# gsgen3d/gsgen

Hardware: AMD Instinct MI355X
Metric: fwd+bwd renders/sec (800x800, 100k Gaussians) (higher is better)
Workload: dtype f32

## Files before the change

gsgen_amd/csrc/common.hpp:

```cpp
#pragma once
#include <hip/hip_runtime.h>
#include <stdint.h>

#if defined(__clang__)
#define GS_WAVES_PER_EU(n) __attribute__((amdgpu_waves_per_eu(n)))
#else
#define GS_WAVES_PER_EU(n)
#endif

namespace gs {

constexpr int kTile = 16;
constexpr int kListOverflow = -2;
constexpr float kMinAlpha = 0.00392156862745098f;
constexpr float kAlphaClamp = 0.99f;
constexpr float kLog2e = 1.4426950408889634f;
constexpr float kGuardTol = 2.0e-4f;
constexpr float kInvSc2 = 1.3862943611198906f;

__device__ __forceinline__ int lane_id() { return (int)(threadIdx.x & 63u); }

struct CholRec { float p0, p1, p2; bool ok; };
__device__ __forceinline__ CholRec chol_prep(float c0, float c1, float c2, float c3) {
#pragma clang fp contract(off)
// ... 14 lines not shown
}

typedef float v2f __attribute__((vector_size(8)));

__device__ __forceinline__ float wave_sum(float v) {
#pragma unroll
  for (int m = 32; m >= 1; m >>= 1) v += __shfl_xor(v, m, 64);
  return v;
}

__device__ __forceinline__ bool wave_any(bool pred) {
#if defined(__HIP_DEVICE_COMPILE__)
  return __builtin_amdgcn_ballot_w64(pred) != 0ull;
#else
  return __ballot((int)pred) != 0ull;
#endif
}
__device__ __forceinline__ void wave_mem_fence() {
#if defined(__HIP_DEVICE_COMPILE__)
  __builtin_amdgcn_fence(__ATOMIC_RELEASE, "workgroup");
  __builtin_amdgcn_wave_barrier();
  __builtin_amdgcn_fence(__ATOMIC_ACQUIRE, "workgroup");
#else
  (void)__ballot(1);
#endif
}
__device__ __forceinline__ float wave_uniform(float v) {
  return __int_as_float(__builtin_amdgcn_readfirstlane(__float_as_int(v)));
}

// ... 346 lines not shown
```

gsgen_amd/csrc/composite.hip:

```cpp
#include "composite_common.hpp"
#include <stdio.h>
#include <string.h>
#include <string>
#include <type_traits>
#include <vector>

namespace gs {

template <int MODE, int CB, int KB = kBatch, bool WITH_COL = true>
struct Stage {
  using TR = Traits<MODE, CB>;
  float mx[KB], my[KB], a[KB];
  float c0[KB], c1[KB], c2[KB], c3[KB];
  float p0[KB], p1[KB], p2[KB];
  int id[KB];
  alignas(16) float col[WITH_COL ? KB * TR::NCOLP : 4];
};

template <int MODE, int CB, int NT, int KB = kBatch, bool SCALE = false, bool WITH_COL = true>
__device__ __forceinline__ void stage_batch(Stage<MODE, CB, KB, WITH_COL> &S, const CompParams &p, int list_base,
                                            int nb) {
  using TR = Traits<MODE, CB>;
  const int t = (int)threadIdx.x;
  static_assert(KB <= NT, "one thread per staged record");
// ... 124 lines not shown
  CompParams v[kPackMax];
  __host__ __device__ const CompParams *table() const { return v; }
};
template <> struct ViewPack<false> {
  __host__ __device__ const CompParams *table() const { return nullptr; }
};
__device__ __forceinline__ uint32_t batch_view(const CompParams &p_arg, uint32_t &bid, uint32_t *grid, uint32_t total) {
  const uint32_t B = (uint32_t)p_arg.n_lo, per = total / B;
  const uint32_t view = bid / per;
  bid -= view * per;
  if (grid) *grid = per;
  return view;
}
__device__ __forceinline__ uint32_t batch_view(const CompParams &p_arg, uint32_t &bid, uint32_t *grid = nullptr) {
  return batch_view(p_arg, bid, grid, gridDim.x);
}

template <int MODE, int CB, int PPL, int TS = 16>
__global__ void __launch_bounds__(TS * TS / PPL) k_composite_fwd(CompParams p) {
  const uint32_t bid = blockIdx.x;
  using TR = Traits<MODE, CB>;
  constexpr int NT = TS * TS / PPL;
  constexpr int ROWS = NT / TS;
  static_assert(TS == 8 || TS == 16 || TS == 32, "tile side");
  static_assert(NT >= kBatch && NT % 64 == 0, "a staging round needs one thread per record");
  constexpr int NCH = TR::NCH;
  __shared__ Stage<MODE, CB> S;

  int tx, ty;
  if (!block_tile(p, tx, ty, bid)) return;
// ... 252 lines not shown
    lg[2][j >> 1][j & 1] = l.s2;
  }
}
template <int NP>
__device__ __forceinline__ void poly_rows_at_pixels(const float *cg, v2f pu2, const v2f (&pv2)[NP], v2f (&yv)[3][NP]) {
#pragma unroll
  for (int c = 0; c < 3; ++c) {
    const float *cw = cg + c * kPolyStride;
    const v2f ab = ffma2(pu2, ffma2(pu2, *reinterpret_cast<const v2f *>(cw + 4), *reinterpret_cast<const v2f *>(cw + 2)),
                         *reinterpret_cast<const v2f *>(cw));
    const float Cc = cw[6];
#pragma unroll
    for (int jp = 0; jp < NP; ++jp) yv[c][jp] = ffma2(pv2[jp], ffma2(pv2[jp], splat2(Cc), splat2(ab[1])), splat2(ab[0]));
  }
}
template <int NT>
__device__ __forceinline__ uint32_t exact_tier_mask(const CompParams &p, const int *ids, int nb, int t, uint32_t *slot) {
  bool bad = false;
  if (p.sh_rows != nullptr && t < nb) bad = !poly_row_ok(p.sh_rows[ids[t]], fmaxf(fabsf(p.psx), fabsf(p.psy)));
  const uint32_t m = (uint32_t)__ballot((int)bad);
  if constexpr (NT == 64) {
    (void)slot;
    return m;
  } else {
    if (t == 0) *slot = m;
    return 0u;
  }
}
template <int CB, bool POLY>
struct FwdShVecShared {
  static constexpr int KB = POLY ? 32 : kBatch;
  Stage<MODE_SH, CB, KB, !POLY> S;
  alignas(16) float Vs[POLY ? kPolyNB * 16 : 4];
  alignas(16) float Ws[POLY ? KB * 3 * kPolyStride : 4];
  uint32_t exact_mask;
  float tay_ok[POLY ? KB * 3 : 1];
};
template <int CB, int PPL, int NB, bool PERSIST = false, bool TRACK = true>
__device__ __forceinline__ void composite_fwd_sh_vec_tile(const CompParams &p, uint32_t bid, FwdShVecShared<CB, (NB > 0)> &sm) {
  static_assert(PPL == 4 || PPL == 2, "pixel pairs: 2 or 4 pixels per lane");
  constexpr bool POLY = NB > 0;
  static_assert(!POLY || (NB == kPolyNB && CB == 4), "polynomial basis: SH degree 3");
  constexpr int MODE = MODE_SH;
  using TR = Traits<MODE, CB>;
  constexpr int NT = 256 / PPL, ROWS = NT / 16, NP = PPL / 2;
  constexpr int CCP = POLY ? NB : TR::CCP, NPAIR = CCP / 2;
  constexpr int KB = FwdShVecShared<CB, POLY>::KB;
  auto &S = sm.S;
  float *const Vs = sm.Vs;
  float *const Ws = sm.Ws;
  int tx, ty;
  if (!block_tile(p, tx, ty, bid)) return;
  const int tile = ty * p.ntw + tx;
  const int st = p.start[tile];
  const int n = (st < 0) ? 0 : (p.end[tile] - st);
  const int t = tile_thread_index<PERSIST>();
  const int lx = t & 15, ly0 = t >> 4;
  const int gx = tx * kTile + lx;

  bool valid[PPL];
  int gy[PPL], stop[PPL];
#pragma unroll
  for (int j = 0; j < PPL; ++j) {
    gy[j] = ty * kTile + ly0 + j * ROWS;
    valid[j] = (gx < p.W) && (gy[j] < p.H);
    stop[j] = valid[j] ? n : 0;
  }
// ... 60 lines not shown
#pragma unroll
  for (int jp = 0; jp < NP; ++jp) {
#pragma unroll
    for (int c = 0; c < 3; ++c) acc2[jp][c] = v2f{0.0f, 0.0f};
    Tr2[jp] = v2f{valid[2 * jp] ? 1.0f : -1.0f, valid[2 * jp + 1] ? 1.0f : -1.0f};
  }
  auto alive = [&](int j) { return !(Tr2[j >> 1][j & 1] < p.thresh); };
  const bool seg_out = p.nseg > 1 && p.ckpt != nullptr;
  const bool track_stop = TRACK && p.stop != nullptr;

  uint32_t exact_mask = 0u;
  uint32_t tay_mask = 0u;
  for (int base = 0; base < n; base += KB) {
    const int nb = min(KB, n - base);
    if (base > 0) __syncthreads();
    stage_batch<MODE, CB, NT, KB, true, !POLY>(S, p, st + base, nb);
    if constexpr (POLY) {
      if (p.sh_rows != nullptr) {
        exact_mask = exact_tier_mask<NT>(p, S.id, nb, t, &sm.exact_mask);
        __syncthreads();
        if constexpr (NT != 64) exact_mask = sm.exact_mask;
        exact_mask = (uint32_t)__builtin_amdgcn_readfirstlane((int)exact_mask);
        if (__popcll((unsigned long long)exact_mask) * kExactTierShare > nb) {
          if (t == 0 && p.route_report != nullptr) report_crowded_tile(p.route_report);
          if (!p.no_fallback) {
            if (t == 0 && p.tile_flags != nullptr) p.tile_flags[tile] = 1;
            return;
          }
        }
      } else {
        exact_mask = 0u;
        __syncthreads();
      }
      poly_transform<NT, KB>(p.col, S.id, Vs, Ws, nb, sm.tay_ok);
      __syncthreads();
      tay_mask = (uint32_t)__builtin_amdgcn_readfirstlane((int)(taylor_mask(sm.tay_ok, nb) & ~exact_mask));
      taylor_convert<NT>(Ws, tay_mask, nb);
      __syncthreads();
    } else {
      __syncthreads();
    }

    for (int g = 0; g < nb; ++g) {
      bool any_alive = false;
#pragma unroll
      for (int j = 0; j < PPL; ++j) any_alive |= alive(j);
      if (!wave_any(any_alive)) break;
      const int e_idx = base + g;
      if (seg_out && (e_idx % kSegLen) == 0 && e_idx > 0 && e_idx / kSegLen < p.nseg) {
#pragma unroll
        for (int j = 0; j < PPL; ++j)
          p.ckpt[((size_t)tile * p.nseg + e_idx / kSegLen) * 256 + (ly0 + j * ROWS) * 16 + lx] =
              make_float4(Tr2[j >> 1][j & 1], acc2[j >> 1][0][j & 1], acc2[j >> 1][1][j & 1], acc2[j >> 1][2][j & 1]);
      }
// ... 186 lines not shown
}
template <int CB, int PPL, bool BATCH = false, int NB = 0, bool TRACK = true, bool PSD = false>
__global__ void __launch_bounds__(256 / PPL)
GS_WAVES_PER_EU((NB == kPolyNB && BATCH && PPL == 4 && !TRACK) ? 5 : 1)
k_composite_fwd_sh_vec(CompParams p_arg, ViewPack<BATCH> pack) {
  static_assert(!PSD || (BATCH && NB != kRouted), "pixel sizes from device memory: the batched launches' three shapes");
  const CompParams *plist = pack.table();
  uint32_t bid = blockIdx.x;
  if constexpr (NB == kRouted) {
    static_assert(CB == 4, "routing exists for SH degree 3");
    union Shared {
      FwdShVecShared<4, true> poly;
      FwdShVecShared<4, false> exact;
    };
    __shared__ Shared sm;
    const CompParams *pp = BATCH ? &plist[batch_view(p_arg, bid)] : &p_arg;
    const bool poly = routed_tile_is_polynomial(*pp, bid);
    if (poly) {
      CompParams p = *pp;
      p.sh_rows = nullptr;
      composite_fwd_sh_vec_tile<4, PPL, kPolyNB>(p, bid, sm.poly);
    } else {
      const CompParams p = *pp;
      composite_fwd_sh_vec_tile<4, PPL, 0>(p, bid, sm.exact);
    }
  } else if constexpr (NB == kFallback) {
    static_assert(CB == 4 && BATCH, "the persistent exact fallback of a bounded batch");
    __shared__ FwdShVecShared<4, false> sm;
    const uint32_t B = (uint32_t)p_arg.n_lo, total = p_arg.vgrid;
    const bool per_tile = plist[0].sh_rows != nullptr;
    if (!per_tile) {
// ... 6 lines not shown
    }
    const uint32_t per = total / B;
    uint32_t base = 0;
    uint32_t view = 0;
    for (uint32_t b = blockIdx.x; b < total; b += gridDim.x) {
      while (b >= base + per) { base += per; ++view; }
      const CompParams *pp = &plist[view];
      const PixelSizes<PSD> ps = view_pixel_sizes<PSD>(*pp);
      if (per_tile ? !tile_flagged(*pp, b - base) : poly_route(pp->sh_bound, ps.x(), ps.y())) continue;
      const CompParams p = view_params<PSD>(*pp, ps);
      composite_fwd_sh_vec_tile<4, PPL, 0, true>(p, b - base, sm);
      __syncthreads();
    }
  } else if constexpr (NB == kPolyNB && BATCH) {
    __shared__ FwdShVecShared<4, true> sm;
    const CompParams *pp = &plist[batch_view(p_arg, bid)];
    const PixelSizes<PSD> ps = view_pixel_sizes<PSD>(*pp);
    const bool view_ok = pp->sh_bound != nullptr && poly_route(pp->sh_bound, ps.x(), ps.y());
    if (pp->sh_rows == nullptr && !view_ok) return;
    CompParams p = view_params<PSD>(*pp, ps);
    if (view_ok) p.sh_rows = nullptr;
    composite_fwd_sh_vec_tile<4, PPL, kPolyNB, false, TRACK>(p, bid, sm);
  } else {
    const CompParams *pp = BATCH ? &plist[batch_view(p_arg, bid)] : &p_arg;
    const CompParams p = view_params<PSD>(*pp, view_pixel_sizes<PSD>(*pp));
    __shared__ FwdShVecShared<CB, (NB > 0)> sm;
    composite_fwd_sh_vec_tile<CB, PPL, NB>(p, bid, sm);
  }
}

template <int MODE, int CB, int PPL, int TS>
__global__ void __launch_bounds__(TS * TS / PPL)
k_composite_bwd_pixel(CompParams p) {
  const uint32_t bid = blockIdx.x, grid = gridDim.x;
  using TR = Traits<MODE, CB>;
  constexpr int NT = TS * TS / PPL;
  static_assert(NT >= kBatch && NT % 64 == 0, "a staging round needs one thread per record");
  constexpr int ROWS = NT / TS;
  constexpr int NCH = TR::NCH;
// ... 207 lines not shown
    for (int j = 0; j < PPL; ++j) any_alive |= alive[j];
    if (__syncthreads_or((int)any_alive) == 0) break;
  }
}


template <int CB, int PPL, bool POLY>
struct BwdShVecShared {
  static constexpr int KB = 32;
  static constexpr int NT = 256 / PPL, NP = PPL / 2;
  Stage<MODE_SH, CB, KB, !POLY> S;
  v2f go_s[!POLY ? 3 * NP * NT : 1];
  alignas(16) float Vs[POLY ? kPolyNB * 16 : 4];
  alignas(16) float Ws[POLY ? KB * 3 * kPolyStride : 4];
  float gw_s[POLY ? 3 * 8 : 1];
  float tay_ok[POLY ? KB * 3 : 1];
};
template <int CB, int PPL, int NB, bool PERSIST = false, bool MOM = false>
__device__ __forceinline__ void composite_bwd_sh_vec_tile(const CompParams &p, uint32_t bid, uint32_t grid,
                                                          BwdShVecShared<CB, PPL, (NB > 0)> &sm) {
  static_assert(PPL == 4 || PPL == 2, "pixel pairs: 2 or 4 pixels per lane");
  constexpr bool POLY = NB > 0;
  static_assert(!POLY || (NB == kPolyNB && CB == 4 && PPL == 4), "polynomial basis: SH degree 3, one wavefront per tile");
  constexpr int MODE = MODE_SH;
  using TR = Traits<MODE, CB>;
  constexpr int NT = 256 / PPL, ROWS = NT / 16, NP = PPL / 2;
  constexpr int CCP = POLY ? NB : TR::CCP, NPAIR = CCP / 2, NSH = 3 * CCP;
  static_assert(NSH % 2 == 0, "component layout");
  constexpr int KB = BwdShVecShared<CB, PPL, POLY>::KB;
  auto &S = sm.S;
  v2f *const go_s = sm.go_s;
  float *const Vs = sm.Vs;
  float *const Ws = sm.Ws;
  float *const gw_s = sm.gw_s;
  const int nseg = p.nseg > 1 ? p.nseg : 1;
  const uint32_t tiles_grid = grid / (uint32_t)nseg;
  const int seg = (int)(bid / tiles_grid);
  int tx, ty;
  if (!block_tile(p, tx, ty, bid % tiles_grid)) return;
  const int tile = ty * p.ntw + tx;
  const int st = p.start[tile];
  const int n = (st < 0) ? 0 : (p.end[tile] - st);
  if (n == 0 || n < p.n_lo || n >= p.n_hi) return;
  if constexpr (POLY) {
    if (p.tile_flags != nullptr && p.tile_flags[tile] != 0) return;
  }
  const int e_lo = seg * kSegLen;
  const int e_hi = (seg == nseg - 1) ? n : min(n, e_lo + kSegLen);
  if (e_lo >= n) return;
  const int t = tile_thread_index<PERSIST>();
  const int lane = t & 63;
  const int lx = t & 15, ly0 = t >> 4;
  const int gx = tx * kTile + lx;
  const float px = pixel_coord(p.topleft[0], gx, p.psx);
// ... 81 lines not shown
    R2[jp] = fma2(go2[jp][2], rem2[jp][2], fma2(go2[jp][1], rem2[jp][1], go2[jp][0] * rem2[jp][0]));
    pvsq2[jp] = pv2[jp] * pv2[jp];
  }
  if constexpr (!POLY) {
#pragma unroll
    for (int jp = 0; jp < NP; ++jp)
#pragma unroll
      for (int c = 0; c < 3; ++c) go_s[(c * NP + jp) * NT + t] = go2[jp][c];
  }
  auto alive = [&](int j) { return !(Tr2[j >> 1][j & 1] < p.thresh); };

  uint32_t exact_mask = 0u, tay_mask = 0u;
  for (int base = e_lo; base < e_hi; base += KB) {
    const int nb = min(KB, e_hi - base);
    if (base > e_lo) __syncthreads();
    stage_batch<MODE, CB, NT, KB, true, !POLY>(S, p, st + base, nb);
    __syncthreads();
    if constexpr (POLY) {
      exact_mask = (uint32_t)__builtin_amdgcn_readfirstlane((int)exact_tier_mask<NT>(p, S.id, nb, t, nullptr));
      poly_transform<NT, KB>(p.col, S.id, Vs, Ws, nb, sm.tay_ok);
      __syncthreads();
      tay_mask = (uint32_t)__builtin_amdgcn_readfirstlane((int)(taylor_mask(sm.tay_ok, nb) & ~exact_mask));
      taylor_convert<NT>(Ws, tay_mask, nb);
      __syncthreads();
    }

    for (int g = 0; g < nb; ++g) {
      bool any_alive = false;
#pragma unroll
      for (int j = 0; j < PPL; ++j) any_alive |= alive(j);
      if (!wave_any(any_alive)) break;

      auto uni = [&](float v) { return !POLY ? wave_uniform(v) : v; };
      const float r_mx = uni(S.mx[g]), r_my = uni(S.my[g]), r_a = uni(S.a[g]), r_c0 = uni(S.c0[g]), r_c1 = uni(S.c1[g]),
                  r_c2 = uni(S.c2[g]), r_c3 = uni(S.c3[g]), r_p0 = uni(S.p0[g]), r_p1 = uni(S.p1[g]);
      const float x = px - r_mx;
      v2f y2[NP], G2[NP], ag2[NP], tx2[NP], ty2[NP];
      bool any_con = false;
      float guard_dist = 0.0f;
#pragma unroll
// ... 224 lines not shown
template <int CB, int PPL, bool BATCH = false, int NB = 0, bool MOM = false, bool PSD = false>
__global__ void __launch_bounds__(256 / PPL)
GS_WAVES_PER_EU((NB == kPolyNB && BATCH) ? 4 : 1)
k_composite_bwd_sh_vec(CompParams p_arg, ViewPack<BATCH> pack) {
  static_assert(!MOM || (BATCH && NB != kRouted), "the moment form exists for the batched launches");
  static_assert(!PSD || (BATCH && NB != kRouted), "pixel sizes from device memory: the batched launches' three shapes");
  const CompParams *plist = pack.table();
  uint32_t bid = blockIdx.x, grid = gridDim.x;
  if constexpr (NB == kRouted) {
    static_assert(CB == 4 && PPL == 4, "routing exists for SH degree 3, one wavefront per tile");
    union Shared {
      BwdShVecShared<4, 4, true> poly;
      BwdShVecShared<4, 4, false> exact;
    };
    __shared__ Shared sm;
    const CompParams *pp = BATCH ? &plist[batch_view(p_arg, bid, &grid)] : &p_arg;
    const uint32_t tiles_grid = grid / (uint32_t)(pp->nseg > 1 ? pp->nseg : 1);
    const bool poly = routed_tile_is_polynomial(*pp, bid % tiles_grid);
    if (poly) {
      CompParams p = *pp;
      p.sh_rows = nullptr;
      composite_bwd_sh_vec_tile<4, 4, kPolyNB>(p, bid, grid, sm.poly);
    } else {
      const CompParams p = *pp;
      composite_bwd_sh_vec_tile<4, 4, 0>(p, bid, grid, sm.exact);
    }
  } else if constexpr (NB == kFallback) {
    static_assert(CB == 4 && PPL == 4 && BATCH, "the persistent exact fallback of a bounded batch");
    __shared__ BwdShVecShared<4, 4, false> sm;
    const uint32_t B = (uint32_t)p_arg.n_lo, total = p_arg.vgrid;
    const bool per_tile = plist[0].sh_rows != nullptr;
// ... 8 lines not shown
    const uint32_t per = total / B;
    const uint32_t tiles_grid = per / (uint32_t)(plist[0].nseg > 1 ? plist[0].nseg : 1);
    uint32_t base = 0;
    uint32_t view = 0;
    for (uint32_t b = blockIdx.x; b < total; b += gridDim.x) {
      while (b >= base + per) { base += per; ++view; }
      const CompParams *pp = &plist[view];
      const PixelSizes<PSD> ps = view_pixel_sizes<PSD>(*pp);
      if (per_tile ? !tile_flagged(*pp, (b - base) % tiles_grid) : poly_route(pp->sh_bound, ps.x(), ps.y())) continue;
      const CompParams p = view_params<PSD>(*pp, ps);
      composite_bwd_sh_vec_tile<4, 4, 0, true, MOM>(p, b - base, per, sm);
      __syncthreads();
    }
  } else if constexpr (NB == kPolyNB && BATCH) {
    __shared__ BwdShVecShared<4, 4, true> sm;
    const CompParams *pp = &plist[batch_view(p_arg, bid, &grid)];
    const PixelSizes<PSD> ps = view_pixel_sizes<PSD>(*pp);
    const bool view_ok = pp->sh_bound != nullptr && poly_route(pp->sh_bound, ps.x(), ps.y());
    if (pp->sh_rows == nullptr && !view_ok) return;
    CompParams p = view_params<PSD>(*pp, ps);
    if (view_ok) p.sh_rows = nullptr;
    composite_bwd_sh_vec_tile<4, 4, kPolyNB, false, MOM>(p, bid, grid, sm);
  } else {
    const CompParams *pp = BATCH ? &plist[batch_view(p_arg, bid, &grid)] : &p_arg;
    const CompParams p = view_params<PSD>(*pp, view_pixel_sizes<PSD>(*pp));
    __shared__ BwdShVecShared<CB, PPL, (NB > 0)> sm;
    composite_bwd_sh_vec_tile<CB, PPL, NB, false, MOM>(p, bid, grid, sm);
  }
}

template <int MODE, bool BATCH = false>
__global__ void __launch_bounds__(64) GS_WAVES_PER_EU(6)
k_composite_fwd_chan_vec(CompParams p_arg, ViewPack<BATCH> pack) {
  const CompParams *plist = pack.table();
  static_assert(MODE == MODE_RGB || MODE == MODE_SCALAR || MODE == MODE_RGBD, "post-activation channel modes");
  uint32_t bid = blockIdx.x;
  const CompParams p = BATCH ? view_params(plist[batch_view(p_arg, bid)]) : p_arg;
  using TR = Traits<MODE, 1>;
  constexpr int PPL = 4, NT = 64, ROWS = NT / 16, NP = PPL / 2;
// ... 402 lines not shown
template <int MODE, int CB>
static int launch_fwd(const CompParams &p_, hipStream_t s) {
  CompParams p = p_;
  const uint32_t nblk = comp_grid(p);
  if (p.ntw * p.nth == 0) return 0;
  if (p.tile_side != 16) {
    if constexpr (MODE == MODE_RGBD) return GSGEN_EUNSUPPORTED;
    else {
      if (p.nseg > 1) return GSGEN_EUNSUPPORTED;
      p.sh_bound = p.sh_rows = nullptr;
      if (p.tile_side == 8) hipLaunchKernelGGL((k_composite_fwd<MODE, CB, 1, 8>), dim3(nblk), dim3(64), 0, s, p);
      else hipLaunchKernelGGL((k_composite_fwd<MODE, CB, 4, 32>), dim3(nblk), dim3(256), 0, s, p);
      return (int)hipGetLastError();
    }
  }
  if constexpr (MODE == MODE_SH && CB == 4) {
    if (p.sh_bound != nullptr || p.sh_rows != nullptr) {
      hipLaunchKernelGGL((k_composite_fwd_sh_vec<4, 2, false, kRouted>), dim3(nblk), dim3(128), 0, s, p, ViewPack<false>{});
      return (int)hipGetLastError();
    }
  } else {
    p.sh_bound = p.sh_rows = nullptr;
  }
  hipLaunchKernelGGL((k_composite_fwd<MODE, CB, 1>), dim3(nblk), dim3(256), 0, s, p);
  return (int)hipGetLastError();
}
template <int MODE, int CB>
static int launch_bwd(const CompParams &p_, hipStream_t s) {
  CompParams p = p_;
  if (p.n_hi == 0) p.n_hi = 0x7fffffff;
  const uint32_t nblk = comp_grid(p);
  if (p.ntw * p.nth == 0) return 0;
  if (p.tile_side != 16) {
    if constexpr (MODE == MODE_RGBD) return GSGEN_EUNSUPPORTED;
    else {
      if (p.nseg > 1) return GSGEN_EUNSUPPORTED;
      p.sh_bound = p.sh_rows = nullptr;
      if (p.tile_side == 8) hipLaunchKernelGGL((k_composite_bwd_pixel<MODE, CB, 1, 8>), dim3(nblk), dim3(64), 0, s, p);
      else hipLaunchKernelGGL((k_composite_bwd_pixel<MODE, CB, 4, 32>), dim3(nblk), dim3(256), 0, s, p);
      return (int)hipGetLastError();
    }
  }
  if constexpr (MODE != MODE_SH) {
    p.sh_bound = nullptr;
    hipLaunchKernelGGL((k_composite_bwd_chan_vec<MODE>), dim3(nblk), dim3(64), 0, s, p, ViewPack<false>{});
  } else {
    const uint32_t ng = nblk * (uint32_t)(p.nseg > 1 ? p.nseg : 1);
    if constexpr (CB == 4) {
      if (p.sh_bound != nullptr || p.sh_rows != nullptr) {
        hipLaunchKernelGGL((k_composite_bwd_sh_vec<4, 4, false, kRouted>), dim3(ng), dim3(64), 0, s, p, ViewPack<false>{});
        return (int)hipGetLastError();
      }
    } else {
      p.sh_bound = p.sh_rows = nullptr;
    }
    hipLaunchKernelGGL((k_composite_bwd_sh_vec<CB, 4>), dim3(ng), dim3(64), 0, s, p, ViewPack<false>{});
  }
  return (int)hipGetLastError();
}


static ViewPack<true> make_pack(const CompParams *host, uint32_t n) {
  ViewPack<true> pack{};
  for (uint32_t i = 0; i < n; ++i) pack.v[i] = host[i];
  return pack;
}
template <class F>
static void for_each_chunk(const CompParams *host, uint32_t B, F &&f) {
  for (uint32_t b0 = 0; b0 < B; b0 += (uint32_t)kPackMax) {
    const uint32_t n = (B - b0) < (uint32_t)kPackMax ? (B - b0) : (uint32_t)kPackMax;
    CompParams a = host[b0];
    a.n_lo = (int)n;
    f(a, make_pack(host + b0, n), n);
  }
}
template <int CB, bool PSD>
static void launch_fwd_sh_batch_c(const CompParams &p0, const ViewPack<true> &plist, uint32_t B, uint32_t nblk, hipStream_t s, bool bounded) {
  const dim3 g(nblk * B);
  if constexpr (CB == 4) {
    if (bounded) {
      CompParams pf = p0;
      pf.vgrid = nblk * B;
      const uint32_t gf = pf.vgrid < 2560u ? pf.vgrid : 2560u;
      const auto fallback = [&] { hipLaunchKernelGGL((k_composite_fwd_sh_vec<4, 2, true, kFallback, true, PSD>), dim3(gf), dim3(128), 0, s, pf, plist); };
      const auto polynomial = [&] {
        if (p0.stop == nullptr) hipLaunchKernelGGL((k_composite_fwd_sh_vec<4, 4, true, kPolyNB, false, PSD>), g, dim3(64), 0, s, p0, plist);
        else hipLaunchKernelGGL((k_composite_fwd_sh_vec<4, 4, true, kPolyNB, true, PSD>), g, dim3(64), 0, s, p0, plist);
// ... 3 lines not shown
        if (!p0.no_fallback) fallback();
        return;
      }
      fallback();
      polynomial();
      return;
    }
  }
  hipLaunchKernelGGL((k_composite_fwd_sh_vec<CB, 2, true, 0, true, PSD>), g, dim3(128), 0, s, p0, plist);
}
template <bool PSD>
static int launch_fwd_sh_batch_p(int C, const CompParams *host, uint32_t B, hipStream_t s, bool bounded) {
  if (B == 0 || host[0].ntw * host[0].nth == 0) return 0;
  const uint32_t nblk = comp_grid(host[0]);
  const bool poly = C == 4 && bounded;
  for_each_chunk(host, B, [&](const CompParams &p0, const ViewPack<true> &pack, uint32_t n) {
    switch (C) {
      case 1: launch_fwd_sh_batch_c<1, PSD>(p0, pack, n, nblk, s, false); break;
      case 2: launch_fwd_sh_batch_c<2, PSD>(p0, pack, n, nblk, s, false); break;
      case 3: launch_fwd_sh_batch_c<3, PSD>(p0, pack, n, nblk, s, false); break;
      default: launch_fwd_sh_batch_c<4, PSD>(p0, pack, n, nblk, s, poly); break;
    }
  });
  return (int)hipGetLastError();
}
int launch_fwd_sh_batch(int C, const CompParams *host, uint32_t B, hipStream_t s, bool bounded) {
  return (B != 0 && host[0].ps_dev != nullptr) ? launch_fwd_sh_batch_p<true>(C, host, B, s, bounded)
                                               : launch_fwd_sh_batch_p<false>(C, host, B, s, bounded);
}
template <int CB, bool MOM, bool PSD>
static void launch_bwd_sh_batch_c(const CompParams &p0, const ViewPack<true> &plist, uint32_t B, uint32_t nblk, hipStream_t s, bool bounded) {
// ... 4 lines not shown
      pf.vgrid = nblk * B;
      const uint32_t gf = pf.vgrid < 3072u ? pf.vgrid : 3072u;
      if (!(p0.sh_rows != nullptr && p0.no_fallback))
        hipLaunchKernelGGL((k_composite_bwd_sh_vec<4, 4, true, kFallback, MOM, PSD>), dim3(gf), dim3(64), 0, s, pf, plist);
      hipLaunchKernelGGL((k_composite_bwd_sh_vec<4, 4, true, kPolyNB, MOM, PSD>), g, dim3(64), 0, s, p0, plist);
      return;
    }
  }
  hipLaunchKernelGGL((k_composite_bwd_sh_vec<CB, 4, true, 0, MOM, PSD>), g, dim3(64), 0, s, p0, plist);
}
template <bool MOM, bool PSD>
static int launch_bwd_sh_batch_m(int C, const CompParams *host, uint32_t B, hipStream_t s, bool bounded) {
  if (B == 0 || host[0].ntw * host[0].nth == 0) return 0;
  const uint32_t nblk = comp_grid(host[0]) * (uint32_t)(host[0].nseg > 1 ? host[0].nseg : 1);
  const bool poly = C == 4 && bounded;
  for_each_chunk(host, B, [&](const CompParams &p0, const ViewPack<true> &pack, uint32_t n) {
    switch (C) {
      case 1: launch_bwd_sh_batch_c<1, MOM, PSD>(p0, pack, n, nblk, s, false); break;
      case 2: launch_bwd_sh_batch_c<2, MOM, PSD>(p0, pack, n, nblk, s, false); break;
      case 3: launch_bwd_sh_batch_c<3, MOM, PSD>(p0, pack, n, nblk, s, false); break;
      default: launch_bwd_sh_batch_c<4, MOM, PSD>(p0, pack, n, nblk, s, poly); break;
    }
  });
  return (int)hipGetLastError();
}
int launch_bwd_sh_batch(int C, const CompParams *host, uint32_t B, hipStream_t s, bool bounded, bool moments = false) {
  if (B != 0 && host[0].ps_dev != nullptr)
    return moments ? launch_bwd_sh_batch_m<true, true>(C, host, B, s, bounded) : launch_bwd_sh_batch_m<false, true>(C, host, B, s, bounded);
  return moments ? launch_bwd_sh_batch_m<true, false>(C, host, B, s, bounded) : launch_bwd_sh_batch_m<false, false>(C, host, B, s, bounded);
}

template <int MODE, bool MOM = false>
static int launch_chan_batch(bool backward, const CompParams *host, uint32_t B, hipStream_t s) {
  if (B == 0 || host[0].ntw * host[0].nth == 0) return 0;
  const uint32_t nblk = comp_grid(host[0]);
  for_each_chunk(host, B, [&](const CompParams &p0, const ViewPack<true> &pack, uint32_t n) {
    if (backward) hipLaunchKernelGGL((k_composite_bwd_chan_vec<MODE, true, MOM>), dim3(nblk * n), dim3(64), 0, s, p0, pack);
    else hipLaunchKernelGGL((k_composite_fwd_chan_vec<MODE, true>), dim3(nblk * n), dim3(64), 0, s, p0, pack);
  });
  return (int)hipGetLastError();
}
int launch_fwd_rgbd_batch(const CompParams *host, uint32_t B, hipStream_t s) { return launch_chan_batch<MODE_RGBD>(false, host, B, s); }
int launch_bwd_rgbd_batch(const CompParams *host, uint32_t B, hipStream_t s) { return launch_chan_batch<MODE_RGBD>(true, host, B, s); }
int launch_bwd_rgbd_batch_moments(const CompParams *host, uint32_t B, hipStream_t s) { return launch_chan_batch<MODE_RGBD, true>(true, host, B, s); }
int launch_fwd_rgb_batch(const CompParams *host, uint32_t B, hipStream_t s) { return launch_chan_batch<MODE_RGB>(false, host, B, s); }
int launch_bwd_rgb_batch(const CompParams *host, uint32_t B, hipStream_t s) { return launch_chan_batch<MODE_RGB>(true, host, B, s); }

int launch_bwd_pixel_dispatch(int mode, int C, const CompParams &p, hipStream_t s) {
  if (mode == MODE_RGB) return launch_bwd<MODE_RGB, 1>(p, s);
  if (mode == MODE_SCALAR) return launch_bwd<MODE_SCALAR, 1>(p, s);
  if (mode == MODE_RGBD) return launch_bwd<MODE_RGBD, 1>(p, s);
// ... 643 lines not shown
```

gsgen_amd/csrc/composite_common.hpp:

```cpp
#pragma once
#include "common.hpp"
#include "../../include/gsgen_hip.h"

namespace gs {

enum : int { MODE_RGB = 0, MODE_SCALAR = 1, MODE_SH = 2, MODE_RGBD = 3 };
constexpr int kBatch = 64;

struct CompParams {
  const float *mean, *cov, *col, *alpha;
  const float *depth;
  const int *start, *end, *ids;
  const float *topleft, *rot, *bg;
  float *out, *T;
  const float *final_img, *grad_out;
  float *g_mean, *g_cov, *g_col, *g_alpha;
  int ntw, nth, H, W;
  float psx, psy, thresh;
  const uint32_t *tile_order;
  int n_lo, n_hi;
  float4 *ckpt;
  int *stop;
  int nseg;
  int tile_side;
  const float *go_rgb, *go_d, *go_o, *go_z2;
  const float *sh_bound;
  const float *sh_rows;
  uint8_t *tile_flags;
  uint32_t vgrid;
  int fill_empty;
  float *pl_rgb, *pl_d, *pl_o, *pl_z;
  float *g_bg;
  int zvar;
  const float *chol;
  uint32_t *route_report;
  int no_fallback;
  const float *ps_dev;
};
__device__ __forceinline__ CompParams view_params(const CompParams &src) {
  CompParams p = src;
  if (p.ps_dev != nullptr) {
    p.psx = p.ps_dev[0];
    p.psy = p.ps_dev[1];
  }
  return p;
}
constexpr int kSegLen = 32;

__device__ __forceinline__ bool block_tile(const CompParams &p, int &tx, int &ty, uint32_t bid) {
  if (p.tile_order != nullptr) {
    const uint32_t t = p.tile_order[bid];
    tx = (int)(t % (uint32_t)p.ntw);
    ty = (int)(t / (uint32_t)p.ntw);
    return true;
  }
  return tile_of_block(bid, p.ntw, p.nth, tx, ty);
}
__device__ __forceinline__ bool block_tile(const CompParams &p, int &tx, int &ty) {
  return block_tile(p, tx, ty, blockIdx.x);
}
__host__ __forceinline__ uint32_t comp_grid(const CompParams &p) {
  return p.tile_order != nullptr ? (uint32_t)(p.ntw * p.nth) : tile_map_blocks(p.ntw, p.nth);
}

static __device__ __noinline__ float gauss_ref_f64(float mx, float my, float c0f, float c1f, float c2f,
                                            float c3f, float px, float py) {
  const double c0 = c0f, c1 = c1f, c2 = c2f, c3 = c3f;
  const double det = c0 * c3 - c1 * c2;
  const double x = (double)(px - mx);
  const double y = (double)(py - my);
  const double tx = x * c3 - y * c2;
  const double ty = -x * c1 + y * c0;
  double radial = tx * x + ty * y;
  radial /= det;
// ... 261 lines not shown
  if (t < 16) {
    float y[kPolyNodes];
#pragma unroll
    for (int n = 0; n < kPolyNodes; ++n) y[n] = Yn[n * 16 + t];
#pragma unroll
    for (int r = 0; r < kPolyNB; ++r) {
      float acc = 0.0f;
#pragma unroll
      for (int n = 0; n < kPolyNodes; ++n)
        if (kPolyFit[r][n] != 0.0f) acc = fmaf(kPolyFit[r][n], y[n], acc);
      Vs[r * 16 + t] = acc;
    }
  }
  __syncthreads();
}
template <int NT, int KB>
__device__ __forceinline__ void poly_transform(const float *__restrict__ sh, const int *ids, const float *Vs, float *w, int nb,
                                               float *tay_ok ) {
  static_assert(NT % 2 == 0, "the two halves of a row sit in neighbouring lanes");
#pragma unroll 1
  for (int it0 = 0; it0 < nb * 6; it0 += NT) {
    const int it = it0 + (int)threadIdx.x;
    const bool live = it < nb * 6;
    const int e = live ? (it >> 1) : 0, half = it & 1;
    const int g = e / 3, c = e - 3 * g;
    const float4 *q4 = reinterpret_cast<const float4 *>(sh + (size_t)ids[g] * 48 + c * 16);
    const float4 q0 = q4[0], q1 = q4[1], q2 = q4[2], q3 = q4[3];
    const v2f qa = {q0.x, q0.y}, qb = {q0.z, q0.w}, qc = {q1.x, q1.y}, qd = {q1.z, q1.w}, qe = {q2.x, q2.y}, qf = {q2.z, q2.w},
              qg = {q3.x, q3.y}, qh = {q3.z, q3.w};
    float *row = w + e * kPolyStride;
    const int s0 = half ? 6 : 0, s1 = half ? 3 : 1, s2 = half ? 4 : 2;
#pragma unroll 1
    for (int k = 0; k < 3; ++k) {
      const float4 *v4 = reinterpret_cast<const float4 *>(Vs + (3 * half + k) * 16);
      const float4 a = v4[0], b = v4[1], cc = v4[2], d = v4[3];
      v2f acc = qa * v2f{a.x, a.y};
      acc = ffma2(qb, v2f{a.z, a.w}, acc);
      acc = ffma2(qc, v2f{b.x, b.y}, acc);
      acc = ffma2(qd, v2f{b.z, b.w}, acc);
      acc = ffma2(qe, v2f{cc.x, cc.y}, acc);
      acc = ffma2(qf, v2f{cc.z, cc.w}, acc);
      acc = ffma2(qg, v2f{d.x, d.y}, acc);
      acc = ffma2(qh, v2f{d.z, d.w}, acc);
      if (live) row[k == 0 ? s0 : (k == 1 ? s1 : s2)] = -kLog2e * (acc[0] + acc[1]);
    }
    if (live && !half) row[5] = 0.0f;
    const float mine = live ? fabsf(row[s0]) + fabsf(row[s1]) + fabsf(row[s2]) : 0.0f;
    const float l1 = xor_add<1>(mine);
    if (live && l1 > 40.0f) {
      const float sc = 40.0f / l1;
      row[s0] *= sc; row[s1] *= sc; row[s2] *= sc;
    }
    if (live && !half) {
      const float l = mine - fabsf(row[0]), q = l1 - mine;
      tay_ok[e] = (l1 <= 40.0f && taylor_row_ok(l, q)) ? 1.0f : 0.0f;
    }
  }
}
template <int NT>
__device__ __forceinline__ void taylor_convert(float *w, uint32_t mask, int nb) {
#pragma unroll 1
  for (int e = (int)threadIdx.x; e < nb * 3; e += NT) {
    if (!((mask >> (e / 3)) & 1u)) continue;
    float *row = w + e * kPolyStride;
    const float w1 = row[1], w2 = row[2], w4 = row[3], w5 = row[4], w3 = row[6];
    const float f0 = __builtin_amdgcn_rcpf(1.0f + __builtin_amdgcn_exp2f(row[0]));
    const float ff = f0 * (1.0f - f0);
    const float f1 = -0.6931471805599453f * ff, f2 = 0.2402265069591007f * ff * (1.0f - 2.0f * f0);
    row[0] = f0;
    row[1] = f1 * w1;
    row[2] = f1 * w2;
    row[3] = fmaf(f1, w4, 2.0f * f2 * w1 * w2);
    row[4] = fmaf(f1, w5, f2 * w2 * w2);
    row[6] = fmaf(f1, w3, f2 * w1 * w1);
  }
}
__device__ __forceinline__ uint32_t taylor_mask(const float *tay_ok, int nb) {
  const int l = lane_id();
  const bool ok = l < nb && tay_ok[3 * l] != 0.0f && tay_ok[3 * l + 1] != 0.0f && tay_ok[3 * l + 2] != 0.0f;
  return (uint32_t)__ballot((int)ok);
}

static inline int check_common(uint32_t tile_size, const void *a, const void *b, const void *c) {
  if (tile_size < 1u || tile_size > 32u) return GSGEN_EUNSUPPORTED;
  if (!a || !b || !c) return GSGEN_EINVAL;
  return 0;
}

}
```

Measured before the change: 7515.

## Fuse polynomial staging, SH transform and Taylor conversion into one wave pass

Replaces the separate stage_batch, exact-tier mask, poly_transform and taylor_convert phases with a single poly_stage_batch. In it, one wavefront handles 32 records using a lane pair per record, and the masks come from ballots instead of shared-memory flags. This removes several __syncthreads barriers and shared-memory round trips per batch. Separately, it precomputes reciprocal multipliers on the host so that block-to-tile and batch-view integer divisions become multiply-shift. The cost is that only 64 threads do the staging work in 128-thread blocks, which may serialize work that was spread before.

New measurement: 7574 (median of 6 runs). Within noise of the previous version (+0.8%).

```diff
diff --git a/gsgen_amd/csrc/common.hpp b/gsgen_amd/csrc/common.hpp
--- a/gsgen_amd/csrc/common.hpp
+++ b/gsgen_amd/csrc/common.hpp
@@ -52,6 +52,13 @@
   return __builtin_amdgcn_ballot_w64(pred) != 0ull;
 #else
   return __ballot((int)pred) != 0ull;
+#endif
+}
+__device__ __forceinline__ unsigned long long wave_ballot(bool pred) {
+#if defined(__HIP_DEVICE_COMPILE__)
+  return __builtin_amdgcn_ballot_w64(pred);
+#else
+  return __ballot((int)pred);
 #endif
 }
 __device__ __forceinline__ void wave_mem_fence() {
diff --git a/gsgen_amd/csrc/composite.hip b/gsgen_amd/csrc/composite.hip
--- a/gsgen_amd/csrc/composite.hip
+++ b/gsgen_amd/csrc/composite.hip
@@ -162,6 +162,14 @@
 }
 __device__ __forceinline__ uint32_t batch_view(const CompParams &p_arg, uint32_t &bid, uint32_t *grid = nullptr) {
   return batch_view(p_arg, bid, grid, gridDim.x);
+}
+__device__ __forceinline__ uint32_t batch_view_rcp(const CompParams &p_arg, uint32_t &bid, uint32_t *grid = nullptr) {
+  if (p_arg.rcp_vper == 0u) return batch_view(p_arg, bid, grid, gridDim.x);
+  const uint32_t per = p_arg.vper;
+  const uint32_t view = div_uniform(bid, per, p_arg.rcp_vper);
+  bid -= view * per;
+  if (grid) *grid = per;
+  return view;
 }
 
 template <int MODE, int CB, int PPL, int TS = 16>
@@ -444,17 +452,82 @@
     for (int jp = 0; jp < NP; ++jp) yv[c][jp] = ffma2(pv2[jp], ffma2(pv2[jp], splat2(Cc), splat2(ab[1])), splat2(ab[0]));
   }
 }
-template <int NT>
-__device__ __forceinline__ uint32_t exact_tier_mask(const CompParams &p, const int *ids, int nb, int t, uint32_t *slot) {
-  bool bad = false;
-  if (p.sh_rows != nullptr && t < nb) bad = !poly_row_ok(p.sh_rows[ids[t]], fmaxf(fabsf(p.psx), fabsf(p.psy)));
-  const uint32_t m = (uint32_t)__ballot((int)bad);
-  if constexpr (NT == 64) {
-    (void)slot;
-    return m;
-  } else {
-    if (t == 0) *slot = m;
-    return 0u;
+template <int NT, int KB>
+__device__ __forceinline__ void poly_stage_batch(Stage<MODE_SH, 4, KB, false> &S, const CompParams &p, const float *Vs, float *Ws,
+                                                 int list_base, int nb, int t, uint32_t &exact_mask, uint32_t &tay_mask,
+                                                 uint32_t *slots) {
+  static_assert(KB == 32 && (NT == 64 || NT == 128), "a lane pair per record: 32 records on one wavefront");
+  if (NT == 64 || t < 64) {
+    const int g = t & 31;
+    const bool half = (t & 32) != 0;
+    const bool live = g < nb;
+    const int id = live ? p.ids[list_base + g] : 0;
+    bool bad = false;
+    if (!half) {
+      float mx = 0.f, my = 0.f, a = 0.f, c0 = 1.f, c1 = 0.f, c2 = 0.f, c3 = 1.f, p0 = 0.f, p1 = 0.f;
+      if (live) {
+        const float2 m = *reinterpret_cast<const float2 *>(p.mean + 2 * (size_t)id);
+        mx = m.x; my = m.y;
+        const float4 c = *reinterpret_cast<const float4 *>(p.cov + 4 * (size_t)id);
+        c0 = c.x; c1 = c.y; c2 = c.z; c3 = c.w;
+        const GRec r = prep_record<MODE_SH>(mx, my, c0, c1, c2, c3, p.alpha[id]);
+        a = r.a; p0 = r.p0; p1 = r.p1;
+      }
+      S.id[g] = id; S.mx[g] = mx; S.my[g] = my; S.a[g] = a;
+      S.c0[g] = c0; S.c1[g] = c1; S.c2[g] = c2; S.c3[g] = c3;
+      S.p0[g] = p0; S.p1[g] = p1; S.p2[g] = 0.f;
+    } else if (p.sh_rows != nullptr && live) {
+      bad = !poly_row_ok(p.sh_rows[id], fmaxf(fabsf(p.psx), fabsf(p.psy)));
+    }
+    const float4 *q4 = reinterpret_cast<const float4 *>(p.col + (size_t)id * 48);
+    const float *vh = Vs + (half ? 3 * 16 : 0);
+    float *row = Ws + g * (3 * kPolyStride);
+    bool tay = live;
+#pragma unroll
+    for (int c = 0; c < 3; ++c) {
+      const float4 q0 = q4[4 * c], q1 = q4[4 * c + 1], q2 = q4[4 * c + 2], q3 = q4[4 * c + 3];
+      const v2f q[8] = {{q0.x, q0.y}, {q0.z, q0.w}, {q1.x, q1.y}, {q1.z, q1.w}, {q2.x, q2.y}, {q2.z, q2.w}, {q3.x, q3.y}, {q3.z, q3.w}};
+      float m0 = poly_monomial(q, vh);
+      __builtin_amdgcn_sched_barrier(0);
+      float m1 = poly_monomial(q, vh + 16);
+      __builtin_amdgcn_sched_barrier(0);
+      float m2 = poly_monomial(q, vh + 32);
+      const float mine = fabsf(m0) + fabsf(m1) + fabsf(m2);
+      const float l1 = xor_add<32>(mine);
+      tay = tay && l1 <= 40.0f && taylor_row_ok(mine - fabsf(m0), l1 - mine);
+      if (l1 > 40.0f) {
+        const float sc = 40.0f / l1;
+        m0 *= sc; m1 *= sc; m2 *= sc;
+      }
+      float *rw = row + c * kPolyStride;
+      if (!half) { rw[0] = m0; rw[1] = m1; rw[2] = m2; rw[5] = 0.0f; }
+      else { rw[6] = m0; rw[3] = m1; rw[4] = m2; }
+    }
+    const uint32_t em = (uint32_t)(wave_ballot(bad) >> 32);
+    const uint32_t tm = (uint32_t)wave_ballot(tay) & ~em;
+    exact_mask = (uint32_t)__builtin_amdgcn_readfirstlane((int)em);
+    tay_mask = (uint32_t)__builtin_amdgcn_readfirstlane((int)tm);
+    if constexpr (NT != 64) {
+      if (t == 0) { slots[0] = exact_mask; slots[1] = tay_mask; }
+    }
+    if (tay_mask != 0u) {
+      wave_mem_fence();
+      float4 w[3];
+      float w5[3], w3[3];
+#pragma unroll
+      for (int c = 0; c < 3; ++c) {
+        const float *rw = row + c * kPolyStride;
+        w[c] = *reinterpret_cast<const float4 *>(rw);
+        w5[c] = rw[4]; w3[c] = rw[6];
+      }
+      wave_mem_fence();
+      if ((tay_mask >> g) & 1u) {
+#pragma unroll
+        for (int c = 0; c < 3; ++c) {
+          taylor_convert_half(row + c * kPolyStride, half, w[c].x, w[c].y, w[c].z, w3[c], w[c].w, w5[c]);
+        }
+      }
+    }
   }
 }
 template <int CB, bool POLY>
@@ -463,8 +536,7 @@
   Stage<MODE_SH, CB, KB, !POLY> S;
   alignas(16) float Vs[POLY ? kPolyNB * 16 : 4];
   alignas(16) float Ws[POLY ? KB * 3 * kPolyStride : 4];
-  uint32_t exact_mask;
-  float tay_ok[POLY ? KB * 3 : 1];
+  uint32_t masks[2];
 };
 template <int CB, int PPL, int NB, bool PERSIST = false, bool TRACK = true>
 __device__ __forceinline__ void composite_fwd_sh_vec_tile(const CompParams &p, uint32_t bid, FwdShVecShared<CB, (NB > 0)> &sm) {
@@ -480,7 +552,7 @@
   float *const Vs = sm.Vs;
   float *const Ws = sm.Ws;
   int tx, ty;
-  if (!block_tile(p, tx, ty, bid)) return;
+  if (!block_tile_rcp(p, tx, ty, bid)) return;
   const int tile = ty * p.ntw + tx;
   const int st = p.start[tile];
   const int n = (st < 0) ? 0 : (p.end[tile] - st);
@@ -571,13 +643,14 @@
   for (int base = 0; base < n; base += KB) {
     const int nb = min(KB, n - base);
     if (base > 0) __syncthreads();
-    stage_batch<MODE, CB, NT, KB, true, !POLY>(S, p, st + base, nb);
     if constexpr (POLY) {
+      poly_stage_batch<NT, KB>(S, p, Vs, Ws, st + base, nb, t, exact_mask, tay_mask, sm.masks);
+      __syncthreads();
+      if constexpr (NT != 64) {
+        exact_mask = p.sh_rows != nullptr ? (uint32_t)__builtin_amdgcn_readfirstlane((int)sm.masks[0]) : 0u;
+        tay_mask = (uint32_t)__builtin_amdgcn_readfirstlane((int)sm.masks[1]);
+      }
       if (p.sh_rows != nullptr) {
-        exact_mask = exact_tier_mask<NT>(p, S.id, nb, t, &sm.exact_mask);
-        __syncthreads();
-        if constexpr (NT != 64) exact_mask = sm.exact_mask;
-        exact_mask = (uint32_t)__builtin_amdgcn_readfirstlane((int)exact_mask);
         if (__popcll((unsigned long long)exact_mask) * kExactTierShare > nb) {
           if (t == 0 && p.route_report != nullptr) report_crowded_tile(p.route_report);
           if (!p.no_fallback) {
@@ -585,16 +658,9 @@
             return;
           }
         }
-      } else {
-        exact_mask = 0u;
-        __syncthreads();
-      }
-      poly_transform<NT, KB>(p.col, S.id, Vs, Ws, nb, sm.tay_ok);
-      __syncthreads();
-      tay_mask = (uint32_t)__builtin_amdgcn_readfirstlane((int)(taylor_mask(sm.tay_ok, nb) & ~exact_mask));
-      taylor_convert<NT>(Ws, tay_mask, nb);
-      __syncthreads();
+      }
     } else {
+      stage_batch<MODE, CB, NT, KB, true, true>(S, p, st + base, nb);
       __syncthreads();
     }
 
@@ -811,7 +877,7 @@
       FwdShVecShared<4, false> exact;
     };
     __shared__ Shared sm;
-    const CompParams *pp = BATCH ? &plist[batch_view(p_arg, bid)] : &p_arg;
+    const CompParams *pp = BATCH ? &plist[batch_view_rcp(p_arg, bid)] : &p_arg;
     const bool poly = routed_tile_is_polynomial(*pp, bid);
     if (poly) {
       CompParams p = *pp;
@@ -848,7 +914,7 @@
     }
   } else if constexpr (NB == kPolyNB && BATCH) {
     __shared__ FwdShVecShared<4, true> sm;
-    const CompParams *pp = &plist[batch_view(p_arg, bid)];
+    const CompParams *pp = &plist[batch_view_rcp(p_arg, bid)];
     const PixelSizes<PSD> ps = view_pixel_sizes<PSD>(*pp);
     const bool view_ok = pp->sh_bound != nullptr && poly_route(pp->sh_bound, ps.x(), ps.y());
     if (pp->sh_rows == nullptr && !view_ok) return;
@@ -856,7 +922,7 @@
     if (view_ok) p.sh_rows = nullptr;
     composite_fwd_sh_vec_tile<4, PPL, kPolyNB, false, TRACK>(p, bid, sm);
   } else {
-    const CompParams *pp = BATCH ? &plist[batch_view(p_arg, bid)] : &p_arg;
+    const CompParams *pp = BATCH ? &plist[batch_view_rcp(p_arg, bid)] : &p_arg;
     const CompParams p = view_params<PSD>(*pp, view_pixel_sizes<PSD>(*pp));
     __shared__ FwdShVecShared<CB, (NB > 0)> sm;
     composite_fwd_sh_vec_tile<CB, PPL, NB>(p, bid, sm);
@@ -1094,7 +1160,6 @@
   alignas(16) float Vs[POLY ? kPolyNB * 16 : 4];
   alignas(16) float Ws[POLY ? KB * 3 * kPolyStride : 4];
   float gw_s[POLY ? 3 * 8 : 1];
-  float tay_ok[POLY ? KB * 3 : 1];
 };
 template <int CB, int PPL, int NB, bool PERSIST = false, bool MOM = false>
 __device__ __forceinline__ void composite_bwd_sh_vec_tile(const CompParams &p, uint32_t bid, uint32_t grid,
@@ -1114,10 +1179,11 @@
   float *const Ws = sm.Ws;
   float *const gw_s = sm.gw_s;
   const int nseg = p.nseg > 1 ? p.nseg : 1;
-  const uint32_t tiles_grid = grid / (uint32_t)nseg;
-  const int seg = (int)(bid / tiles_grid);
+  const bool rcp = p.rcp_tgrid != 0u;
+  const uint32_t tiles_grid = rcp ? p.tgrid : grid / (uint32_t)nseg;
+  const int seg = (int)(rcp ? div_uniform(bid, tiles_grid, p.rcp_tgrid) : bid / tiles_grid);
   int tx, ty;
-  if (!block_tile(p, tx, ty, bid % tiles_grid)) return;
+  if (!block_tile_rcp(p, tx, ty, bid - (uint32_t)seg * tiles_grid)) return;
   const int tile = ty * p.ntw + tx;
   const int st = p.start[tile];
   const int n = (st < 0) ? 0 : (p.end[tile] - st);
@@ -1229,16 +1295,13 @@
   for (int base = e_lo; base < e_hi; base += KB) {
     const int nb = min(KB, e_hi - base);
     if (base > e_lo) __syncthreads();
-    stage_batch<MODE, CB, NT, KB, true, !POLY>(S, p, st + base, nb);
+    if constexpr (POLY) {
+      static_assert(!POLY || NT == 64, "one wavefront per tile");
+      poly_stage_batch<NT, KB>(S, p, Vs, Ws, st + base, nb, t, exact_mask, tay_mask, nullptr);
+    } else {
+      stage_batch<MODE, CB, NT, KB, true, true>(S, p, st + base, nb);
+    }
     __syncthreads();
-    if constexpr (POLY) {
-      exact_mask = (uint32_t)__builtin_amdgcn_readfirstlane((int)exact_tier_mask<NT>(p, S.id, nb, t, nullptr));
-      poly_transform<NT, KB>(p.col, S.id, Vs, Ws, nb, sm.tay_ok);
-      __syncthreads();
-      tay_mask = (uint32_t)__builtin_amdgcn_readfirstlane((int)(taylor_mask(sm.tay_ok, nb) & ~exact_mask));
-      taylor_convert<NT>(Ws, tay_mask, nb);
-      __syncthreads();
-    }
 
     for (int g = 0; g < nb; ++g) {
       bool any_alive = false;
@@ -1493,7 +1556,7 @@
       BwdShVecShared<4, 4, false> exact;
     };
     __shared__ Shared sm;
-    const CompParams *pp = BATCH ? &plist[batch_view(p_arg, bid, &grid)] : &p_arg;
+    const CompParams *pp = BATCH ? &plist[batch_view_rcp(p_arg, bid, &grid)] : &p_arg;
     const uint32_t tiles_grid = grid / (uint32_t)(pp->nseg > 1 ? pp->nseg : 1);
     const bool poly = routed_tile_is_polynomial(*pp, bid % tiles_grid);
     if (poly) {
@@ -1532,7 +1595,7 @@
     }
   } else if constexpr (NB == kPolyNB && BATCH) {
     __shared__ BwdShVecShared<4, 4, true> sm;
-    const CompParams *pp = &plist[batch_view(p_arg, bid, &grid)];
+    const CompParams *pp = &plist[batch_view_rcp(p_arg, bid, &grid)];
     const PixelSizes<PSD> ps = view_pixel_sizes<PSD>(*pp);
     const bool view_ok = pp->sh_bound != nullptr && poly_route(pp->sh_bound, ps.x(), ps.y());
     if (pp->sh_rows == nullptr && !view_ok) return;
@@ -1540,7 +1603,7 @@
     if (view_ok) p.sh_rows = nullptr;
     composite_bwd_sh_vec_tile<4, 4, kPolyNB, false, MOM>(p, bid, grid, sm);
   } else {
-    const CompParams *pp = BATCH ? &plist[batch_view(p_arg, bid, &grid)] : &p_arg;
+    const CompParams *pp = BATCH ? &plist[batch_view_rcp(p_arg, bid, &grid)] : &p_arg;
     const CompParams p = view_params<PSD>(*pp, view_pixel_sizes<PSD>(*pp));
     __shared__ BwdShVecShared<CB, PPL, (NB > 0)> sm;
     composite_bwd_sh_vec_tile<CB, PPL, NB, false, MOM>(p, bid, grid, sm);
@@ -1973,6 +2036,7 @@
       return (int)hipGetLastError();
     }
   }
+  if constexpr (MODE == MODE_SH) set_tile_divisors(p);
   if constexpr (MODE == MODE_SH && CB == 4) {
     if (p.sh_bound != nullptr || p.sh_rows != nullptr) {
       hipLaunchKernelGGL((k_composite_fwd_sh_vec<4, 2, false, kRouted>), dim3(nblk), dim3(128), 0, s, p, ViewPack<false>{});
@@ -2000,6 +2064,7 @@
       return (int)hipGetLastError();
     }
   }
+  if constexpr (MODE == MODE_SH) set_tile_divisors(p);
   if constexpr (MODE != MODE_SH) {
     p.sh_bound = nullptr;
     hipLaunchKernelGGL((k_composite_bwd_chan_vec<MODE>), dim3(nblk), dim3(64), 0, s, p, ViewPack<false>{});
@@ -2021,15 +2086,20 @@
 
 static ViewPack<true> make_pack(const CompParams *host, uint32_t n) {
   ViewPack<true> pack{};
-  for (uint32_t i = 0; i < n; ++i) pack.v[i] = host[i];
+  for (uint32_t i = 0; i < n; ++i) {
+    pack.v[i] = host[i];
+    set_tile_divisors(pack.v[i]);
+  }
   return pack;
 }
 template <class F>
-static void for_each_chunk(const CompParams *host, uint32_t B, F &&f) {
+static void for_each_chunk(const CompParams *host, uint32_t B, uint32_t per, F &&f) {
   for (uint32_t b0 = 0; b0 < B; b0 += (uint32_t)kPackMax) {
     const uint32_t n = (B - b0) < (uint32_t)kPackMax ? (B - b0) : (uint32_t)kPackMax;
     CompParams a = host[b0];
     a.n_lo = (int)n;
+    a.vper = per;
+    a.rcp_vper = rcp_word(per, (uint64_t)per * n);
     f(a, make_pack(host + b0, n), n);
   }
 }
@@ -2063,7 +2133,7 @@
   if (B == 0 || host[0].ntw * host[0].nth == 0) return 0;
   const uint32_t nblk = comp_grid(host[0]);
   const bool poly = C == 4 && bounded;
-  for_each_chunk(host, B, [&](const CompParams &p0, const ViewPack<true> &pack, uint32_t n) {
+  for_each_chunk(host, B, nblk, [&](const CompParams &p0, const ViewPack<true> &pack, uint32_t n) {
     switch (C) {
       case 1: launch_fwd_sh_batch_c<1, PSD>(p0, pack, n, nblk, s, false); break;
       case 2: launch_fwd_sh_batch_c<2, PSD>(p0, pack, n, nblk, s, false); break;
@@ -2098,7 +2168,7 @@
   if (B == 0 || host[0].ntw * host[0].nth == 0) return 0;
   const uint32_t nblk = comp_grid(host[0]) * (uint32_t)(host[0].nseg > 1 ? host[0].nseg : 1);
   const bool poly = C == 4 && bounded;
-  for_each_chunk(host, B, [&](const CompParams &p0, const ViewPack<true> &pack, uint32_t n) {
+  for_each_chunk(host, B, nblk, [&](const CompParams &p0, const ViewPack<true> &pack, uint32_t n) {
     switch (C) {
       case 1: launch_bwd_sh_batch_c<1, MOM, PSD>(p0, pack, n, nblk, s, false); break;
       case 2: launch_bwd_sh_batch_c<2, MOM, PSD>(p0, pack, n, nblk, s, false); break;
@@ -2118,7 +2188,7 @@
 static int launch_chan_batch(bool backward, const CompParams *host, uint32_t B, hipStream_t s) {
   if (B == 0 || host[0].ntw * host[0].nth == 0) return 0;
   const uint32_t nblk = comp_grid(host[0]);
-  for_each_chunk(host, B, [&](const CompParams &p0, const ViewPack<true> &pack, uint32_t n) {
+  for_each_chunk(host, B, nblk, [&](const CompParams &p0, const ViewPack<true> &pack, uint32_t n) {
     if (backward) hipLaunchKernelGGL((k_composite_bwd_chan_vec<MODE, true, MOM>), dim3(nblk * n), dim3(64), 0, s, p0, pack);
     else hipLaunchKernelGGL((k_composite_fwd_chan_vec<MODE, true>), dim3(nblk * n), dim3(64), 0, s, p0, pack);
   });
diff --git a/gsgen_amd/csrc/composite_common.hpp b/gsgen_amd/csrc/composite_common.hpp
--- a/gsgen_amd/csrc/composite_common.hpp
+++ b/gsgen_amd/csrc/composite_common.hpp
@@ -36,7 +36,17 @@
   uint32_t *route_report;
   int no_fallback;
   const float *ps_dev;
+  uint32_t rcp_ntw, rcp_sw, tgrid, rcp_tgrid, vper, rcp_vper;
 };
+__host__ __forceinline__ uint32_t rcp_word(uint32_t d, uint64_t nmax) {
+  if (d < 2u || nmax * (uint64_t)d >= (1ull << 32)) return 0u;
+  return (uint32_t)(((1ull << 32) + d - 1u) / d);
+}
+__device__ __forceinline__ uint32_t div_uniform(uint32_t n, uint32_t d, uint32_t rcp) {
+  n = (uint32_t)__builtin_amdgcn_readfirstlane((int)n);
+  if (rcp != 0u) return (uint32_t)(((uint64_t)n * (uint64_t)rcp) >> 32);
+  return n / d;
+}
 __device__ __forceinline__ CompParams view_params(const CompParams &src) {
   CompParams p = src;
   if (p.ps_dev != nullptr) {
@@ -58,6 +68,33 @@
 }
 __device__ __forceinline__ bool block_tile(const CompParams &p, int &tx, int &ty) {
   return block_tile(p, tx, ty, blockIdx.x);
+}
+__device__ __forceinline__ bool block_tile_rcp(const CompParams &p, int &tx, int &ty, uint32_t bid) {
+  if (p.tile_order != nullptr) {
+    const uint32_t t = p.tile_order[bid];
+    const uint32_t q = div_uniform(t, (uint32_t)p.ntw, p.rcp_ntw);
+    tx = (int)(t - q * (uint32_t)p.ntw);
+    ty = (int)q;
+    return true;
+  }
+  const uint32_t xcd = bid & 7u, idx = bid >> 3;
+  const uint32_t j = idx >> 4, k = idx & 15u;
+  const uint32_t sw = (uint32_t)((p.ntw + 3) >> 2), sh = (uint32_t)((p.nth + 3) >> 2);
+  const uint32_t sidx = xcd + 8u * j;
+  if (sidx >= sw * sh) return false;
+  const uint32_t q = div_uniform(sidx, sw, p.rcp_sw);
+  tx = (int)((sidx - q * sw) * 4u + (k & 3u));
+  ty = (int)(q * 4u + (k >> 2));
+  return tx < p.ntw && ty < p.nth;
+}
+__host__ __forceinline__ void set_tile_divisors(CompParams &p) {
+  const uint32_t ntw = (uint32_t)p.ntw, nth = (uint32_t)p.nth;
+  const uint32_t sw = (ntw + 3u) >> 2, sh = (nth + 3u) >> 2;
+  const uint32_t nseg = p.nseg > 1 ? (uint32_t)p.nseg : 1u;
+  p.rcp_ntw = rcp_word(ntw, (uint64_t)ntw * nth);
+  p.rcp_sw = rcp_word(sw, (uint64_t)sw * sh + 7u);
+  p.tgrid = p.tile_order != nullptr ? ntw * nth : tile_map_blocks(p.ntw, p.nth);
+  p.rcp_tgrid = rcp_word(p.tgrid, (uint64_t)p.tgrid * nseg);
 }
 __host__ __forceinline__ uint32_t comp_grid(const CompParams &p) {
   return p.tile_order != nullptr ? (uint32_t)(p.ntw * p.nth) : tile_map_blocks(p.ntw, p.nth);
@@ -349,71 +386,32 @@
   }
   __syncthreads();
 }
-template <int NT, int KB>
-__device__ __forceinline__ void poly_transform(const float *__restrict__ sh, const int *ids, const float *Vs, float *w, int nb,
-                                               float *tay_ok ) {
-  static_assert(NT % 2 == 0, "the two halves of a row sit in neighbouring lanes");
-#pragma unroll 1
-  for (int it0 = 0; it0 < nb * 6; it0 += NT) {
-    const int it = it0 + (int)threadIdx.x;
-    const bool live = it < nb * 6;
-    const int e = live ? (it >> 1) : 0, half = it & 1;
-    const int g = e / 3, c = e - 3 * g;
-    const float4 *q4 = reinterpret_cast<const float4 *>(sh + (size_t)ids[g] * 48 + c * 16);
-    const float4 q0 = q4[0], q1 = q4[1], q2 = q4[2], q3 = q4[3];
-    const v2f qa = {q0.x, q0.y}, qb = {q0.z, q0.w}, qc = {q1.x, q1.y}, qd = {q1.z, q1.w}, qe = {q2.x, q2.y}, qf = {q2.z, q2.w},
-              qg = {q3.x, q3.y}, qh = {q3.z, q3.w};
-    float *row = w + e * kPolyStride;
-    const int s0 = half ? 6 : 0, s1 = half ? 3 : 1, s2 = half ? 4 : 2;
-#pragma unroll 1
-    for (int k = 0; k < 3; ++k) {
-      const float4 *v4 = reinterpret_cast<const float4 *>(Vs + (3 * half + k) * 16);
-      const float4 a = v4[0], b = v4[1], cc = v4[2], d = v4[3];
-      v2f acc = qa * v2f{a.x, a.y};
-      acc = ffma2(qb, v2f{a.z, a.w}, acc);
-      acc = ffma2(qc, v2f{b.x, b.y}, acc);
-      acc = ffma2(qd, v2f{b.z, b.w}, acc);
-      acc = ffma2(qe, v2f{cc.x, cc.y}, acc);
-      acc = ffma2(qf, v2f{cc.z, cc.w}, acc);
-      acc = ffma2(qg, v2f{d.x, d.y}, acc);
-      acc = ffma2(qh, v2f{d.z, d.w}, acc);
-      if (live) row[k == 0 ? s0 : (k == 1 ? s1 : s2)] = -kLog2e * (acc[0] + acc[1]);
-    }
-    if (live && !half) row[5] = 0.0f;
-    const float mine = live ? fabsf(row[s0]) + fabsf(row[s1]) + fabsf(row[s2]) : 0.0f;
-    const float l1 = xor_add<1>(mine);
-    if (live && l1 > 40.0f) {
-      const float sc = 40.0f / l1;
-      row[s0] *= sc; row[s1] *= sc; row[s2] *= sc;
-    }
-    if (live && !half) {
-      const float l = mine - fabsf(row[0]), q = l1 - mine;
-      tay_ok[e] = (l1 <= 40.0f && taylor_row_ok(l, q)) ? 1.0f : 0.0f;
-    }
-  }
-}
-template <int NT>
-__device__ __forceinline__ void taylor_convert(float *w, uint32_t mask, int nb) {
-#pragma unroll 1
-  for (int e = (int)threadIdx.x; e < nb * 3; e += NT) {
-    if (!((mask >> (e / 3)) & 1u)) continue;
-    float *row = w + e * kPolyStride;
-    const float w1 = row[1], w2 = row[2], w4 = row[3], w5 = row[4], w3 = row[6];
-    const float f0 = __builtin_amdgcn_rcpf(1.0f + __builtin_amdgcn_exp2f(row[0]));
-    const float ff = f0 * (1.0f - f0);
-    const float f1 = -0.6931471805599453f * ff, f2 = 0.2402265069591007f * ff * (1.0f - 2.0f * f0);
+__device__ __forceinline__ float poly_monomial(const v2f (&q)[8], const float *v) {
+  const float4 *v4 = reinterpret_cast<const float4 *>(v);
+  const float4 a = v4[0], b = v4[1], cc = v4[2], d = v4[3];
+  v2f acc = q[0] * v2f{a.x, a.y};
+  acc = ffma2(q[1], v2f{a.z, a.w}, acc);
+  acc = ffma2(q[2], v2f{b.x, b.y}, acc);
+  acc = ffma2(q[3], v2f{b.z, b.w}, acc);
+  acc = ffma2(q[4], v2f{cc.x, cc.y}, acc);
+  acc = ffma2(q[5], v2f{cc.z, cc.w}, acc);
+  acc = ffma2(q[6], v2f{d.x, d.y}, acc);
+  acc = ffma2(q[7], v2f{d.z, d.w}, acc);
+  return -kLog2e * (acc[0] + acc[1]);
+}
+__device__ __forceinline__ void taylor_convert_half(float *row, bool half, float w0, float w1, float w2, float w3, float w4, float w5) {
+  const float f0 = __builtin_amdgcn_rcpf(1.0f + __builtin_amdgcn_exp2f(w0));
+  const float ff = f0 * (1.0f - f0);
+  const float f1 = -0.6931471805599453f * ff, f2 = 0.2402265069591007f * ff * (1.0f - 2.0f * f0);
+  if (!half) {
     row[0] = f0;
     row[1] = f1 * w1;
     row[2] = f1 * w2;
+  } else {
     row[3] = fmaf(f1, w4, 2.0f * f2 * w1 * w2);
     row[4] = fmaf(f1, w5, f2 * w2 * w2);
     row[6] = fmaf(f1, w3, f2 * w1 * w1);
   }
-}
-__device__ __forceinline__ uint32_t taylor_mask(const float *tay_ok, int nb) {
-  const int l = lane_id();
-  const bool ok = l < nb && tay_ok[3 * l] != 0.0f && tay_ok[3 * l + 1] != 0.0f && tay_ok[3 * l + 2] != 0.0f;
-  return (uint32_t)__ballot((int)ok);
 }
 
 static inline int check_common(uint32_t tile_size, const void *a, const void *b, const void *c) {
```
